# mayataka/idocp

Measured on AMD Instinct MI355X. Metric: SQP iterations/sec (whole node), higher is better.
Workload: dtype f64; 1 GPU; ANYmal OCPSolver N=100 T=5.05 FP64, trotting contact sequence (1 lift + 9 impulse events, 120 stages incl. impulse / aux / lift stages, switching constraints; BASELINE.json configs[2]); batch=1024 independent OCP instances per GPU, replicas across GPUs; horizon=100, batch_per_gpu=1024, parallelism=replicas x1

## Files before the change

### idocp_amd/csrc/ocp_nominal_kernel.hip

```cpp
#include <hip/hip_runtime.h>

#include "dev_dense.hpp"
#include "dev_lie.hpp"
#include "dev_rnea_tangent.hpp"
#include "ocp_device.hpp"
#include "ocp_launch.hpp"

namespace idocp_dev {

namespace {
using namespace rt;
__device__ __forceinline__ void st3g(double* __restrict__ p, V3 a) { p[0] = a.x; p[1] = a.y; p[2] = a.z; }
}

template <typename D, bool XYY, bool IMP>
__global__ __launch_bounds__(64) void ocp_nominal_kernel(OcpBuffers B, int dbg, int nlist, const double* __restrict__ q0) {
  using L = OcpLayout<D>;
  constexpr int NL = D::NL, LJ = D::LJ, NV = D::NV;
  constexpr int NOUT = 30, NIN = L::NJ_DYN - NOUT, TS = 31;
  __shared__ double tr[64 * TS];
  __shared__ long long recs[64];
  const OcpProblem* __restrict__ P = B.prob;
  const DevModel* __restrict__ m = B.model;
  const int M = B.M;
  const int lane = threadIdx.x;
  const int NTASK = 2 * NL + 1 + ((!IMP && q0 != nullptr) ? 3 : 0);
  const unsigned n_blk = blockIdx.x;
  const unsigned g_lo = n_blk & 7u, tg = n_blk >> 3;
  const unsigned g_hi = tg / NTASK;
  const int task = (int)(tg - g_hi * NTASK);
  const long unit = (long)(g_hi * 8u + g_lo) * 64 + lane;
  const int per = IMP ? nlist : M;
  const bool in_range = unit < (long)P->batch * per;
  const long b = in_range ? unit / per : 0;
  const int pos = in_range ? (IMP ? B.impulse_pos[(int)(unit - b * per)] : (int)(unit - b * per)) : (IMP ? B.impulse_pos[0] : 0);
  const OcpNode* __restrict__ nd = B.nodes + pos;
  const bool valid = in_range && pos != M - 1 && (IMP || nd->kind != 1);
  const long rec = (dbg & 2) ? 0 : b * B.NS + nd->slot;
  const double* __restrict__ s = B.sol + rec * L::SOL;
  double* __restrict__ nom = B.nom + rec * L::NOM;
  const double gz = IMP ? 0.0 : m->gravity[2];
  const double wv = 2.0 / P->baumgarte_time_step, wp = 1.0 / (P->baumgarte_time_step * P->baumgarte_time_step);
  const double* __restrict__ sq = s + L::S_Q;
  const double* __restrict__ sv = s + L::S_V;
  const double* __restrict__ sa = s + L::S_A;
  const double qx = sq[3], qy = sq[4], qz = sq[5], qw = sq[6];

  if (!IMP && task > 2 * NL) {
    if (!in_range) return;
    const int lt = task - 2 * NL - 1;
    double* __restrict__ zz = B.lie + rec * L::LIE;
    double R[9], p[3], Ja[36], Jb[36], d6[6];
    if (lt == 0) {
      lieRelative(B.q_ref + (long)pos * D::NQ, sq, R, p);
      lieLog6(R, p, d6);
      lieJlog6(R, p, Ja);
      for (int k = 0; k < 36; ++k) zz[L::Z_JQ + k] = Ja[k];
      for (int k = 0; k < 6; ++k) zz[L::Z_QDIFF + k] = d6[k];
    } else if (lt == 1) {
      if (pos == M - 1) return;
      lieRelative(B.sol + (b * B.NS + nd->next) * L::SOL + L::S_Q, sq, R, p);
      lieLog6(R, p, d6);
      lieJlog6(R, p, Ja);
      for (int k = 0; k < 36; ++k) zz[L::Z_FQQ + k] = Ja[k];
      for (int k = 0; k < 6; ++k) zz[L::Z_FQ6 + k] = d6[k];
      lieDDiffArg0(R, p, Ja, Jb);
      lieBlockInverse(Jb, Ja);
      for (int k = 0; k < 36; ++k) zz[L::Z_FQQI + k] = Ja[k];
    } else {
      const double* __restrict__ q_prev = (nd->prev < 0) ? (q0 + b * D::NQ) : (B.sol + (b * B.NS + nd->prev) * L::SOL + L::S_Q);
      lieRelative(sq, q_prev, R, p);
      lieJlog6(R, p, Ja);
      lieDDiffArg0(R, p, Ja, Jb);
      for (int k = 0; k < 36; ++k) zz[L::Z_FQQP + k] = Jb[k];
      lieBlockInverse(Jb, Ja);
      for (int k = 0; k < 36; ++k) zz[L::Z_FQQPI + k] = Ja[k];
    }
    return;
  }
  if (task <= NL) {
    const V3 zb = v3(2 * (qx * qz - qy * qw), 2 * (qy * qz + qx * qw), 1 - 2 * (qx * qx + qy * qy));
    V3 v = IMP ? ld3(sv) + ld3(sa) : ld3(sv), w = IMP ? ld3(sv + 3) + ld3(sa + 3) : ld3(sv + 3);
    V3 bl = ld3(sa) - gz * zb, bw = ld3(sa + 3);
    if (task == NL) {
      if (!valid) return;
      V3 hl = v3(0, 0, 0), hn = hl, f, n;
      const V3 mc = ld3(m->mc[0]);
      if (!IMP) inertia(m->mass[0], mc, m->Io[0], v, w, hl, hn);
      inertia(m->mass[0], mc, m->Io[0], bl, bw, f, n);
      double* br = nom + L::O_BASE;
      st3g(br + 0, zb); st3g(br + 3, v); st3g(br + 6, w); st3g(br + 9, hl); st3g(br + 12, hn); br[15] = 0.0;
      double* bn = nom + L::O_BN;
      if (IMP) { st3g(bn, f); st3g(bn + 3, n); }
      else { st3g(bn, f + cross(w, hl)); st3g(bn + 3, n + cross(w, hn) + cross(v, hl)); }
      double* idc = nom + L::O_IDC;
#pragma unroll
      for (int r = 0; r < 6; ++r) idc[r] = 0.0;
      for (int r = NV + nd->dimf; r < L::NVF; ++r) idc[r] = 0.0;
      return;
    }
    const int leg = task;
    recs[lane] = valid ? (long long)rec : -1;
    auto flush = [&](auto ncols, int offset) {
      constexpr int N = decltype(ncols)::value;
      waveLdsSync();
#pragma unroll 6
      for (int i = 0; i < N; ++i) {
        const int f = 64 * i + lane, st = f / N, k = f - st * N;
        const long long r = recs[st];
        if (r >= 0 && !(dbg & 1)) B.nom[r * L::NOM + offset + k] = tr[st * TS + k];
      }
      waveLdsSync();
    };
    double* my = tr + lane * TS;
    double Rj[LJ][12];
    V3 wj[LJ], vj[LJ], bwj[LJ], blj[LJ];
    V3 zc = zb;
#pragma unroll
    for (int j = 0; j < LJ; ++j) {
      const int ji = 1 + leg * LJ + j, dof = 6 + leg * LJ + j;
      double sj, cj;
      sincos(sq[dof + 1], &sj, &cj);
      Mat3<double> Rm;
      revoluteRotation<double>(m->R[ji], m->axis[ji], cj, sj, Rm);
#pragma unroll
      for (int e = 0; e < 9; ++e) Rj[j][e] = Rm.m[e];
      const V3 u = ld3(m->axis[ji]), p = ld3(m->p[ji]);
      st3(&Rj[j][9], u);
      const double qdd = sa[dof], qd = IMP ? sv[dof] + qdd : sv[dof];
      V3 wc, vc, bwc, blc, vJ;
      auto step = [&](auto tag) {
        const JointFrame<decltype(tag)::value> F(Rj[j], 0, 9);
        wc = F.mulT(w); vc = F.mulT(v + cross(w, p)); bwc = F.mulT(bw); blc = F.mulT(bl + cross(bw, p));
        zc = F.mulT(zc);
        vJ = F.timesU(qd);
        w = wc + vJ; v = vc;
        if constexpr (IMP) { bw = bwc + F.timesU(qdd); bl = blc; }
        else {
          bw = bwc + F.timesU(qdd) + F.crossKU(w, qd);
          bl = blc + F.crossKU(v, qd);
        }
      };
      if constexpr (XYY) { if (j == 0) step(AxisTag<0>{}); else step(AxisTag<1>{}); } else step(AxisTag<-1>{});
      wj[j] = w; vj[j] = v; bwj[j] = bw; blj[j] = bl;
#pragma unroll
      for (int e = 0; e < 9; ++e) my[e] = Rj[j][e];
      st3(my + 9, wc); st3(my + 12, vc); st3(my + 15, bwc); st3(my + 18, blc); st3(my + 21, zc); st3(my + 24, vJ); st3(my + 27, w);
      flush(AxisTag<NOUT>{}, L::O_JOINT + (leg * LJ + j) * L::NJ_DYN);
    }
    double* fr = nom + L::O_FEET + leg * L::NF_DYN;
    V3 fel = v3(0, 0, 0), fen = fel, fv = fel, fw = fel;
    double* idc = nom + L::O_IDC;
    if (valid && nd->active[leg]) {
      const double* __restrict__ Rc = P->contact_R[leg];
      const V3 pc = ld3(P->contact_p[leg]);
      const int row = NV + nd->row_of[leg];
      fv = XYY ? v + cross(w, pc) : mulT(Rc, v + cross(w, pc)); fw = XYY ? w : mulT(Rc, w);
      if constexpr (IMP) {
        idc[row] = fv.x; idc[row + 1] = fv.y; idc[row + 2] = fv.z;
      } else {
        const V3 fam = XYY ? bl + cross(bw, pc) : mulT(Rc, bl + cross(bw, pc));
        const V3 wxv = cross(fw, fv);
        idc[row] = fam.x + wxv.x + wv * fv.x;
        idc[row + 1] = fam.y + wxv.y + wv * fv.y;
        idc[row + 2] = fam.z + wxv.z + wv * fv.z;
      }
      fel = XYY ? ld3(s + L::S_F + 3 * leg) : mul(Rc, ld3(s + L::S_F + 3 * leg));
      fen = cross(pc, fel);
    }
    if (valid) { st3g(fr + 9, fv); st3g(fr + 12, fw); }
    V3 Fl = v3(0, 0, 0) - fel, Fn = v3(0, 0, 0) - fen;
#pragma unroll
    for (int j = LJ - 1; j >= 0; --j) {
      const int ji = 1 + leg * LJ + j, dof = 6 + leg * LJ + j;
      const V3 p = ld3(m->p[ji]), mc = ld3(m->mc[ji]);
      V3 hl = v3(0, 0, 0), hn = hl, f, n;
      inertia(m->mass[ji], mc, m->Io[ji], blj[j], bwj[j], f, n);
      if constexpr (IMP) { Fl = Fl + f; Fn = Fn + n; }
      else {
        inertia(m->mass[ji], mc, m->Io[ji], vj[j], wj[j], hl, hn);
        Fl = Fl + f + cross(wj[j], hl);
        Fn = Fn + n + cross(wj[j], hn) + cross(vj[j], hl);
      }
      st3(my, hl); st3(my + 3, hn); st3(my + 6, Fl); st3(my + 9, Fn);
      flush(AxisTag<NIN>{}, L::O_JOINT + (leg * LJ + j) * L::NJ_DYN + NOUT);
      auto back = [&](auto tag) {
        const JointFrame<decltype(tag)::value> F(Rj[j], 0, 9);
        if (valid) idc[dof] = F.dotU(Fn);
        const V3 Rf = F.mul(Fl);
        Fn = F.mul(Fn) + cross(p, Rf);
        Fl = Rf;
      };
      if constexpr (XYY) { if (j == 0) back(AxisTag<0>{}); else back(AxisTag<1>{}); } else back(AxisTag<-1>{});
    }
    if (valid) { double* bn = nom + L::O_BN + 6 * (1 + leg); st3g(bn, Fl); st3g(bn + 3, Fn); }
    return;
  }
  if (!valid) return;
  const int leg = task - NL - 1;
  double* fr = nom + L::O_FEET + leg * L::NF_DYN;
  V3 cp = v3(0, 0, 0);
  double rwc[9];
#pragma unroll
  for (int e = 0; e < 9; ++e) rwc[e] = 0.0;
  if (!IMP && nd->active[leg]) {
    double Rw[9];
    Rw[0] = 1 - 2 * (qy * qy + qz * qz); Rw[1] = 2 * (qx * qy - qz * qw);     Rw[2] = 2 * (qx * qz + qy * qw);
    Rw[3] = 2 * (qx * qy + qz * qw);     Rw[4] = 1 - 2 * (qx * qx + qz * qz); Rw[5] = 2 * (qy * qz - qx * qw);
    Rw[6] = 2 * (qx * qz - qy * qw);     Rw[7] = 2 * (qy * qz + qx * qw);     Rw[8] = 1 - 2 * (qx * qx + qy * qy);
    V3 pw = ld3(sq);
#pragma unroll
    for (int j = 0; j < LJ; ++j) {
      const int ji = 1 + leg * LJ + j, dof = 6 + leg * LJ + j;
      double sj, cj;
      sincos(sq[dof + 1], &sj, &cj);
      Mat3<double> Rm;
      revoluteRotation<double>(m->R[ji], m->axis[ji], cj, sj, Rm);
      pw = pw + mul(Rw, ld3(m->p[ji]));
      double Rl[12];
#pragma unroll
      for (int e = 0; e < 9; ++e) Rl[e] = Rm.m[e];
      st3(&Rl[9], ld3(m->axis[ji]));
      auto turn = [&](auto tag) {
        const JointFrame<decltype(tag)::value> F(Rl, 0, 9);
#pragma unroll
        for (int r = 0; r < 3; ++r) {
          const V3 row = F.mulT(v3(Rw[3 * r], Rw[3 * r + 1], Rw[3 * r + 2]));
          Rw[3 * r] = row.x; Rw[3 * r + 1] = row.y; Rw[3 * r + 2] = row.z;
        }
      };
      if constexpr (XYY) { if (j == 0) turn(AxisTag<0>{}); else turn(AxisTag<1>{}); } else turn(AxisTag<-1>{});
    }
    const double* __restrict__ Rc = P->contact_R[leg];
    const V3 pf = pw + mul(Rw, ld3(P->contact_p[leg]));
#pragma unroll
    for (int r = 0; r < 3; ++r)
#pragma unroll
      for (int c = 0; c < 3; ++c) rwc[3 * r + c] = XYY ? Rw[3 * r + c] : Rw[3 * r] * Rc[c] + Rw[3 * r + 1] * Rc[3 + c] + Rw[3 * r + 2] * Rc[6 + c];
    const V3 g = XYY ? gz * v3(Rw[6], Rw[7], Rw[8]) : mulT(Rc, gz * v3(Rw[6], Rw[7], Rw[8]));
    cp = v3(g.x + wp * (pf.x - nd->contact_point[leg][0]), g.y + wp * (pf.y - nd->contact_point[leg][1]),
            g.z + wp * (pf.z - nd->contact_point[leg][2]));
  }
#pragma unroll
  for (int e = 0; e < 9; ++e) fr[e] = rwc[e];
  st3g(fr + 15, cp);
}

template <typename D>
void OcpLaunch<D>::nominal(const OcpBuffers& B, long batch, int M, hipStream_t st, const double* q0_lie, hipStream_t st_imp) {
  const unsigned ntask = 2 * D::NL + 1 + (q0_lie ? 3 : 0);
  const unsigned groups = (unsigned)((batch * M + 63) / 64), blocks = ((groups + 7) / 8) * 8 * ntask;
  if (B.leg_axes_xyy) hipLaunchKernelGGL((ocp_nominal_kernel<D, true, false>), dim3(blocks), dim3(64), 0, st, B, 0, 0, q0_lie);
  else hipLaunchKernelGGL((ocp_nominal_kernel<D, false, false>), dim3(blocks), dim3(64), 0, st, B, 0, 0, q0_lie);
  if (B.n_impulse_fe > 0) {
    const unsigned gi = (unsigned)((batch * B.n_impulse_fe + 63) / 64), bi = ((gi + 7) / 8) * 8 * (2 * D::NL + 1);
    const double* none = nullptr;
    hipStream_t si = st_imp ? st_imp : st;
    if (B.leg_axes_xyy) hipLaunchKernelGGL((ocp_nominal_kernel<D, true, true>), dim3(bi), dim3(64), 0, si, B, 0, B.n_impulse_fe, none);
    else hipLaunchKernelGGL((ocp_nominal_kernel<D, false, true>), dim3(bi), dim3(64), 0, si, B, 0, B.n_impulse_fe, none);
  }
}

template void OcpLaunch<LeggedDims<4, 3>>::nominal(const OcpBuffers&, long, int, hipStream_t, const double*, hipStream_t);

}
```

Before: 212,500 SQP iterations/s.

## Coalesce nominal kernel loads/stores via LDS transposition and merge leg tasks

Loads of the per-stage solution (q, v, a, joint states, forces) and all scattered per-thread global stores (base record, feet, idc rows, Lie Jacobians) now go through a wave-level LDS transpose, so each wave issues contiguous loads and 16-byte stores. The separate foot-kinematics task is merged into the leg RNEA task, which cuts the task count from 2*NL+1 to NL+1 and removes duplicated sincos and rotation work. The price is more LDS traffic and barriers, higher register pressure in the merged leg task, and alignment static_asserts on the record layout.

```diff
diff --git a/idocp_amd/csrc/ocp_nominal_kernel.hip b/idocp_amd/csrc/ocp_nominal_kernel.hip
--- a/idocp_amd/csrc/ocp_nominal_kernel.hip
+++ b/idocp_amd/csrc/ocp_nominal_kernel.hip
@@ -10,21 +10,56 @@
 
 namespace {
 using namespace rt;
-__device__ __forceinline__ void st3g(double* __restrict__ p, V3 a) { p[0] = a.x; p[1] = a.y; p[2] = a.z; }
+
+template <int S, int N, bool W16>
+__device__ __forceinline__ void trStore(const double* col0, const int* recs, unsigned long long live, double* __restrict__ out, int reclen, int offset, int lane) {
+  static_assert(!W16 || N % 2 == 0, "16-byte runs have an even length");
+  constexpr int W = W16 ? 2 : 1, NW = N / W;
+#pragma unroll 6
+  for (int i = 0; i < NW; ++i) {
+    const int e = 64 * i + lane, st = e / NW, k = W * (e - st * NW);
+    if (!((live >> st) & 1ull)) continue;
+    double* __restrict__ dst = out + (long)recs[st] * reclen + offset + k;
+    if constexpr (W16) *reinterpret_cast<double2*>(dst) = make_double2(col0[st * S + k], col0[st * S + k + 1]);
+    else *dst = col0[st * S + k];
+  }
+}
+template <int S, int N>
+__device__ __forceinline__ void trStoreAt(const double* col0, const int* recs, const int* at, unsigned long long live, double* __restrict__ out, int reclen, int offset, int lane) {
+#pragma unroll
+  for (int i = 0; i < N; ++i) {
+    const int e = 64 * i + lane, st = e / N, k = e - st * N;
+    if (((live >> st) & 1ull) && at[st] >= 0) out[(long)recs[st] * reclen + offset + at[st] + k] = col0[st * S + k];
+  }
+}
+template <int S, int N>
+__device__ __forceinline__ void trLoad(double* col0, const int* recs, const double* __restrict__ in, int reclen, int offset, int lane) {
+#pragma unroll
+  for (int i = 0; i < N; ++i) {
+    const int e = 64 * i + lane, st = e / N, k = e - st * N;
+    col0[st * S + k] = in[(long)recs[st] * reclen + offset + k];
+  }
+}
 }
 
 template <typename D, bool XYY, bool IMP>
 __global__ __launch_bounds__(64) void ocp_nominal_kernel(OcpBuffers B, int dbg, int nlist, const double* __restrict__ q0) {
   using L = OcpLayout<D>;
-  constexpr int NL = D::NL, LJ = D::LJ, NV = D::NV;
+  constexpr int NL = D::NL, LJ = D::LJ, NV = D::NV, NF = D::NF;
   constexpr int NOUT = 30, NIN = L::NJ_DYN - NOUT, TS = 31;
-  __shared__ double tr[64 * TS];
-  __shared__ long long recs[64];
+  static_assert(L::NOM % 2 == 0 && L::LIE % 2 == 0 && L::O_JOINT % 2 == 0 && L::NJ_DYN % 2 == 0 && NOUT % 2 == 0 && L::O_FEET % 2 == 0 && L::NF_DYN % 2 == 0 &&
+                L::O_BASE % 2 == 0 && L::NB_DYN % 2 == 0 && L::O_BN % 2 == 0, "16-byte stores of the nominal record");
+  static_assert(L::Z_JQ % 2 == 0 && L::Z_FQQ % 2 == 0 && L::Z_FQQI % 2 == 0 && L::Z_FQQP % 2 == 0, "16-byte stores of the Lie record");
+  static_assert(L::Z_QDIFF == L::Z_JQ + 36 && L::Z_FQ6 == L::Z_FQQ + 36 && L::Z_FQQPI == L::Z_FQQP + 36, "neighbouring Lie blocks leave as one run");
+  static_assert(L::O_BN == L::O_BASE + L::NB_DYN && L::NB_DYN == 16, "base record and own base force leave as one run");
+  static_assert(L::NF_DYN == 18 && 16 + 3 * LJ <= TS && L::NF_DYN + 3 <= TS && 6 + LJ <= TS, "rows of the leg task");
+  __shared__ __attribute__((aligned(16))) double tr[64 * TS];
+  __shared__ int recs[64], aux[64];
   const OcpProblem* __restrict__ P = B.prob;
   const DevModel* __restrict__ m = B.model;
   const int M = B.M;
   const int lane = threadIdx.x;
-  const int NTASK = 2 * NL + 1 + ((!IMP && q0 != nullptr) ? 3 : 0);
+  const int NTASK = NL + 1 + ((!IMP && q0 != nullptr) ? 3 : 0);
   const unsigned n_blk = blockIdx.x;
   const unsigned g_lo = n_blk & 7u, tg = n_blk >> 3;
   const unsigned g_hi = tg / NTASK;
@@ -37,223 +72,266 @@
   const OcpNode* __restrict__ nd = B.nodes + pos;
   const bool valid = in_range && pos != M - 1 && (IMP || nd->kind != 1);
   const long rec = (dbg & 2) ? 0 : b * B.NS + nd->slot;
-  const double* __restrict__ s = B.sol + rec * L::SOL;
-  double* __restrict__ nom = B.nom + rec * L::NOM;
+  const unsigned long long store_on = (dbg & 1) ? 0ull : ~0ull;
   const double gz = IMP ? 0.0 : m->gravity[2];
   const double wv = 2.0 / P->baumgarte_time_step, wp = 1.0 / (P->baumgarte_time_step * P->baumgarte_time_step);
-  const double* __restrict__ sq = s + L::S_Q;
-  const double* __restrict__ sv = s + L::S_V;
-  const double* __restrict__ sa = s + L::S_A;
-  const double qx = sq[3], qy = sq[4], qz = sq[5], qw = sq[6];
-
-  if (!IMP && task > 2 * NL) {
-    if (!in_range) return;
-    const int lt = task - 2 * NL - 1;
-    double* __restrict__ zz = B.lie + rec * L::LIE;
+  recs[lane] = (int)rec;
+  double* my = tr + lane * TS;
+  auto put = [&](auto k0_, auto n_, auto get, unsigned long long live, double* __restrict__ out, int reclen, int offset) {
+    constexpr int K0 = decltype(k0_)::value, N = decltype(n_)::value, S = N | 1;
+    static_assert(N <= TS - 1 && K0 % 2 == 0, "a block fits the transposition; runs stay 16-byte aligned");
+#pragma unroll
+    for (int k = 0; k < N; ++k) tr[lane * S + k] = get(K0 + k);
+    waveLdsSync();
+    trStore<S, N, true>(tr, recs, live, out, reclen, offset + K0, lane);
+    waveLdsSync();
+  };
+
+  if (!IMP && task > NL) {
+    const int lt = task - NL - 1;
+    constexpr int SQ = 7;
+    waveLdsSync();
+    trLoad<SQ, 7>(tr, recs, B.sol, L::SOL, L::S_Q, lane);
+    waveLdsSync();
+    double sq[7];
+#pragma unroll
+    for (int k = 0; k < 7; ++k) sq[k] = tr[lane * SQ + k];
+    waveLdsSync();
     double R[9], p[3], Ja[36], Jb[36], d6[6];
+    auto JaD6 = [&](int k) { return k < 36 ? Ja[k] : d6[k - 36]; };
+    auto JaOnly = [&](int k) { return Ja[k]; };
+    auto JbJa = [&](int k) { return k < 36 ? Jb[k] : Ja[k - 36]; };
     if (lt == 0) {
+      const unsigned long long live = __ballot(in_range) & store_on;
       lieRelative(B.q_ref + (long)pos * D::NQ, sq, R, p);
       lieLog6(R, p, d6);
       lieJlog6(R, p, Ja);
-      for (int k = 0; k < 36; ++k) zz[L::Z_JQ + k] = Ja[k];
-      for (int k = 0; k < 6; ++k) zz[L::Z_QDIFF + k] = d6[k];
+      put(AxisTag<0>{}, AxisTag<22>{}, JaD6, live, B.lie, L::LIE, L::Z_JQ);
+      put(AxisTag<22>{}, AxisTag<20>{}, JaD6, live, B.lie, L::LIE, L::Z_JQ);
     } else if (lt == 1) {
-      if (pos == M - 1) return;
-      lieRelative(B.sol + (b * B.NS + nd->next) * L::SOL + L::S_Q, sq, R, p);
+      const bool on = in_range && pos != M - 1;
+      const unsigned long long live = __ballot(on) & store_on;
+      lieRelative(B.sol + (b * B.NS + (on ? nd->next : nd->slot)) * L::SOL + L::S_Q, sq, R, p);
       lieLog6(R, p, d6);
       lieJlog6(R, p, Ja);
-      for (int k = 0; k < 36; ++k) zz[L::Z_FQQ + k] = Ja[k];
-      for (int k = 0; k < 6; ++k) zz[L::Z_FQ6 + k] = d6[k];
+      put(AxisTag<0>{}, AxisTag<22>{}, JaD6, live, B.lie, L::LIE, L::Z_FQQ);
+      put(AxisTag<22>{}, AxisTag<20>{}, JaD6, live, B.lie, L::LIE, L::Z_FQQ);
       lieDDiffArg0(R, p, Ja, Jb);
       lieBlockInverse(Jb, Ja);
-      for (int k = 0; k < 36; ++k) zz[L::Z_FQQI + k] = Ja[k];
+      put(AxisTag<0>{}, AxisTag<18>{}, JaOnly, live, B.lie, L::LIE, L::Z_FQQI);
+      put(AxisTag<18>{}, AxisTag<18>{}, JaOnly, live, B.lie, L::LIE, L::Z_FQQI);
     } else {
+      const unsigned long long live = __ballot(in_range) & store_on;
       const double* __restrict__ q_prev = (nd->prev < 0) ? (q0 + b * D::NQ) : (B.sol + (b * B.NS + nd->prev) * L::SOL + L::S_Q);
       lieRelative(sq, q_prev, R, p);
       lieJlog6(R, p, Ja);
       lieDDiffArg0(R, p, Ja, Jb);
-      for (int k = 0; k < 36; ++k) zz[L::Z_FQQP + k] = Jb[k];
       lieBlockInverse(Jb, Ja);
-      for (int k = 0; k < 36; ++k) zz[L::Z_FQQPI + k] = Ja[k];
+      put(AxisTag<0>{}, AxisTag<24>{}, JbJa, live, B.lie, L::LIE, L::Z_FQQP);
+      put(AxisTag<24>{}, AxisTag<24>{}, JbJa, live, B.lie, L::LIE, L::Z_FQQP);
+      put(AxisTag<48>{}, AxisTag<24>{}, JbJa, live, B.lie, L::LIE, L::Z_FQQP);
     }
     return;
   }
-  if (task <= NL) {
-    const V3 zb = v3(2 * (qx * qz - qy * qw), 2 * (qy * qz + qx * qw), 1 - 2 * (qx * qx + qy * qy));
-    V3 v = IMP ? ld3(sv) + ld3(sa) : ld3(sv), w = IMP ? ld3(sv + 3) + ld3(sa + 3) : ld3(sv + 3);
-    V3 bl = ld3(sa) - gz * zb, bw = ld3(sa + 3);
-    if (task == NL) {
-      if (!valid) return;
-      V3 hl = v3(0, 0, 0), hn = hl, f, n;
-      const V3 mc = ld3(m->mc[0]);
-      if (!IMP) inertia(m->mass[0], mc, m->Io[0], v, w, hl, hn);
-      inertia(m->mass[0], mc, m->Io[0], bl, bw, f, n);
-      double* br = nom + L::O_BASE;
-      st3g(br + 0, zb); st3g(br + 3, v); st3g(br + 6, w); st3g(br + 9, hl); st3g(br + 12, hn); br[15] = 0.0;
-      double* bn = nom + L::O_BN;
-      if (IMP) { st3g(bn, f); st3g(bn + 3, n); }
-      else { st3g(bn, f + cross(w, hl)); st3g(bn + 3, n + cross(w, hn) + cross(v, hl)); }
-      double* idc = nom + L::O_IDC;
-#pragma unroll
-      for (int r = 0; r < 6; ++r) idc[r] = 0.0;
-      for (int r = NV + nd->dimf; r < L::NVF; ++r) idc[r] = 0.0;
-      return;
-    }
-    const int leg = task;
-    recs[lane] = valid ? (long long)rec : -1;
-    auto flush = [&](auto ncols, int offset) {
-      constexpr int N = decltype(ncols)::value;
-      waveLdsSync();
-#pragma unroll 6
-      for (int i = 0; i < N; ++i) {
-        const int f = 64 * i + lane, st = f / N, k = f - st * N;
-        const long long r = recs[st];
-        if (r >= 0 && !(dbg & 1)) B.nom[r * L::NOM + offset + k] = tr[st * TS + k];
-      }
-      waveLdsSync();
-    };
-    double* my = tr + lane * TS;
-    double Rj[LJ][12];
-    V3 wj[LJ], vj[LJ], bwj[LJ], blj[LJ];
-    V3 zc = zb;
-#pragma unroll
-    for (int j = 0; j < LJ; ++j) {
-      const int ji = 1 + leg * LJ + j, dof = 6 + leg * LJ + j;
-      double sj, cj;
-      sincos(sq[dof + 1], &sj, &cj);
-      Mat3<double> Rm;
-      revoluteRotation<double>(m->R[ji], m->axis[ji], cj, sj, Rm);
-#pragma unroll
-      for (int e = 0; e < 9; ++e) Rj[j][e] = Rm.m[e];
-      const V3 u = ld3(m->axis[ji]), p = ld3(m->p[ji]);
-      st3(&Rj[j][9], u);
-      const double qdd = sa[dof], qd = IMP ? sv[dof] + qdd : sv[dof];
-      V3 wc, vc, bwc, blc, vJ;
-      auto step = [&](auto tag) {
-        const JointFrame<decltype(tag)::value> F(Rj[j], 0, 9);
-        wc = F.mulT(w); vc = F.mulT(v + cross(w, p)); bwc = F.mulT(bw); blc = F.mulT(bl + cross(bw, p));
-        zc = F.mulT(zc);
-        vJ = F.timesU(qd);
-        w = wc + vJ; v = vc;
-        if constexpr (IMP) { bw = bwc + F.timesU(qdd); bl = blc; }
-        else {
-          bw = bwc + F.timesU(qdd) + F.crossKU(w, qd);
-          bl = blc + F.crossKU(v, qd);
-        }
-      };
-      if constexpr (XYY) { if (j == 0) step(AxisTag<0>{}); else step(AxisTag<1>{}); } else step(AxisTag<-1>{});
-      wj[j] = w; vj[j] = v; bwj[j] = bw; blj[j] = bl;
-#pragma unroll
-      for (int e = 0; e < 9; ++e) my[e] = Rj[j][e];
-      st3(my + 9, wc); st3(my + 12, vc); st3(my + 15, bwc); st3(my + 18, blc); st3(my + 21, zc); st3(my + 24, vJ); st3(my + 27, w);
-      flush(AxisTag<NOUT>{}, L::O_JOINT + (leg * LJ + j) * L::NJ_DYN);
-    }
-    double* fr = nom + L::O_FEET + leg * L::NF_DYN;
-    V3 fel = v3(0, 0, 0), fen = fel, fv = fel, fw = fel;
-    double* idc = nom + L::O_IDC;
-    if (valid && nd->active[leg]) {
-      const double* __restrict__ Rc = P->contact_R[leg];
-      const V3 pc = ld3(P->contact_p[leg]);
-      const int row = NV + nd->row_of[leg];
-      fv = XYY ? v + cross(w, pc) : mulT(Rc, v + cross(w, pc)); fw = XYY ? w : mulT(Rc, w);
-      if constexpr (IMP) {
-        idc[row] = fv.x; idc[row + 1] = fv.y; idc[row + 2] = fv.z;
-      } else {
-        const V3 fam = XYY ? bl + cross(bw, pc) : mulT(Rc, bl + cross(bw, pc));
-        const V3 wxv = cross(fw, fv);
-        idc[row] = fam.x + wxv.x + wv * fv.x;
-        idc[row + 1] = fam.y + wxv.y + wv * fv.y;
-        idc[row + 2] = fam.z + wxv.z + wv * fv.z;
-      }
-      fel = XYY ? ld3(s + L::S_F + 3 * leg) : mul(Rc, ld3(s + L::S_F + 3 * leg));
-      fen = cross(pc, fel);
-    }
-    if (valid) { st3g(fr + 9, fv); st3g(fr + 12, fw); }
-    V3 Fl = v3(0, 0, 0) - fel, Fn = v3(0, 0, 0) - fen;
-#pragma unroll
-    for (int j = LJ - 1; j >= 0; --j) {
-      const int ji = 1 + leg * LJ + j, dof = 6 + leg * LJ + j;
-      const V3 p = ld3(m->p[ji]), mc = ld3(m->mc[ji]);
-      V3 hl = v3(0, 0, 0), hn = hl, f, n;
-      inertia(m->mass[ji], mc, m->Io[ji], blj[j], bwj[j], f, n);
-      if constexpr (IMP) { Fl = Fl + f; Fn = Fn + n; }
-      else {
-        inertia(m->mass[ji], mc, m->Io[ji], vj[j], wj[j], hl, hn);
-        Fl = Fl + f + cross(wj[j], hl);
-        Fn = Fn + n + cross(wj[j], hn) + cross(vj[j], hl);
-      }
-      st3(my, hl); st3(my + 3, hn); st3(my + 6, Fl); st3(my + 9, Fn);
-      flush(AxisTag<NIN>{}, L::O_JOINT + (leg * LJ + j) * L::NJ_DYN + NOUT);
-      auto back = [&](auto tag) {
-        const JointFrame<decltype(tag)::value> F(Rj[j], 0, 9);
-        if (valid) idc[dof] = F.dotU(Fn);
-        const V3 Rf = F.mul(Fl);
-        Fn = F.mul(Fn) + cross(p, Rf);
-        Fl = Rf;
-      };
-      if constexpr (XYY) { if (j == 0) back(AxisTag<0>{}); else back(AxisTag<1>{}); } else back(AxisTag<-1>{});
-    }
-    if (valid) { double* bn = nom + L::O_BN + 6 * (1 + leg); st3g(bn, Fl); st3g(bn + 3, Fn); }
+  const unsigned long long live = __ballot(valid) & store_on;
+  const int leg = task < NL ? task : 0;
+  constexpr int C_V = 7, C_A = 13, C_QJ = 19, C_VJ = C_QJ + LJ, C_AJ = C_VJ + LJ, C_F = C_AJ + LJ;
+  waveLdsSync();
+  trLoad<TS, 7>(tr, recs, B.sol, L::SOL, L::S_Q, lane);
+  trLoad<TS, 6>(tr + C_V, recs, B.sol, L::SOL, L::S_V, lane);
+  trLoad<TS, 6>(tr + C_A, recs, B.sol, L::SOL, L::S_A, lane);
+  if (task < NL) {
+    trLoad<TS, LJ>(tr + C_QJ, recs, B.sol, L::SOL, L::S_Q + 7 + leg * LJ, lane);
+    trLoad<TS, LJ>(tr + C_VJ, recs, B.sol, L::SOL, L::S_V + 6 + leg * LJ, lane);
+    trLoad<TS, LJ>(tr + C_AJ, recs, B.sol, L::SOL, L::S_A + 6 + leg * LJ, lane);
+    trLoad<TS, 3>(tr + C_F, recs, B.sol, L::SOL, L::S_F + 3 * leg, lane);
+  }
+  waveLdsSync();
+  double sq[7], sv[6], sa[6];
+#pragma unroll
+  for (int k = 0; k < 7; ++k) sq[k] = my[k];
+#pragma unroll
+  for (int k = 0; k < 6; ++k) { sv[k] = my[C_V + k]; sa[k] = my[C_A + k]; }
+  const double qx = sq[3], qy = sq[4], qz = sq[5], qw = sq[6];
+  const V3 zb = v3(2 * (qx * qz - qy * qw), 2 * (qy * qz + qx * qw), 1 - 2 * (qx * qx + qy * qy));
+  V3 v = IMP ? ld3(sv) + ld3(sa) : ld3(sv), w = IMP ? ld3(sv + 3) + ld3(sa + 3) : ld3(sv + 3);
+  V3 bl = ld3(sa) - gz * zb, bw = ld3(sa + 3);
+  if (task == NL) {
+    waveLdsSync();
+    V3 hl = v3(0, 0, 0), hn = hl, f, n;
+    const V3 mc = ld3(m->mc[0]);
+    if (!IMP) inertia(m->mass[0], mc, m->Io[0], v, w, hl, hn);
+    inertia(m->mass[0], mc, m->Io[0], bl, bw, f, n);
+    constexpr int SB = (L::NB_DYN + 6) | 1;
+    double* br = tr + lane * SB;
+    st3(br + 0, zb); st3(br + 3, v); st3(br + 6, w); st3(br + 9, hl); st3(br + 12, hn); br[15] = 0.0;
+    double* bn = br + L::NB_DYN;
+    if (IMP) { st3(bn, f); st3(bn + 3, n); }
+    else { st3(bn, f + cross(w, hl)); st3(bn + 3, n + cross(w, hn) + cross(v, hl)); }
+    aux[lane] = nd->dimf;
+    waveLdsSync();
+    trStore<SB, L::NB_DYN + 6, true>(tr, recs, live, B.nom, L::NOM, L::O_BASE, lane);
+#pragma unroll
+    for (int i = 0; i < 6; ++i) {
+      const int e = 64 * i + lane, st = e / 6, k = e - st * 6;
+      if ((live >> st) & 1ull) B.nom[(long)recs[st] * L::NOM + L::O_IDC + k] = 0.0;
+    }
+#pragma unroll
+    for (int i = 0; i < NF; ++i) {
+      const int e = 64 * i + lane, st = e / NF, k = e - st * NF;
+      if (((live >> st) & 1ull) && k >= aux[st]) B.nom[(long)recs[st] * L::NOM + L::O_IDC + NV + k] = 0.0;
+    }
     return;
   }
-  if (!valid) return;
-  const int leg = task - NL - 1;
-  double* fr = nom + L::O_FEET + leg * L::NF_DYN;
-  V3 cp = v3(0, 0, 0);
-  double rwc[9];
-#pragma unroll
-  for (int e = 0; e < 9; ++e) rwc[e] = 0.0;
-  if (!IMP && nd->active[leg]) {
-    double Rw[9];
+  double qj[LJ], qdj[LJ], qddj[LJ];
+#pragma unroll
+  for (int j = 0; j < LJ; ++j) { qj[j] = my[C_QJ + j]; qdj[j] = my[C_VJ + j]; qddj[j] = my[C_AJ + j]; }
+  const V3 fs = ld3(my + C_F);
+  waveLdsSync();
+  auto flush = [&](auto ncols, int offset) {
+    constexpr int N = decltype(ncols)::value;
+    waveLdsSync();
+    trStore<TS, N, true>(tr, recs, live, B.nom, L::NOM, offset, lane);
+    waveLdsSync();
+  };
+  double Rj[LJ][12];
+  V3 wj[LJ], vj[LJ], bwj[LJ], blj[LJ];
+  V3 zc = zb;
+  double Rw[9];
+  V3 pw = ld3(sq);
+  if constexpr (!IMP) {
     Rw[0] = 1 - 2 * (qy * qy + qz * qz); Rw[1] = 2 * (qx * qy - qz * qw);     Rw[2] = 2 * (qx * qz + qy * qw);
     Rw[3] = 2 * (qx * qy + qz * qw);     Rw[4] = 1 - 2 * (qx * qx + qz * qz); Rw[5] = 2 * (qy * qz - qx * qw);
     Rw[6] = 2 * (qx * qz - qy * qw);     Rw[7] = 2 * (qy * qz + qx * qw);     Rw[8] = 1 - 2 * (qx * qx + qy * qy);
-    V3 pw = ld3(sq);
-#pragma unroll
-    for (int j = 0; j < LJ; ++j) {
-      const int ji = 1 + leg * LJ + j, dof = 6 + leg * LJ + j;
-      double sj, cj;
-      sincos(sq[dof + 1], &sj, &cj);
-      Mat3<double> Rm;
-      revoluteRotation<double>(m->R[ji], m->axis[ji], cj, sj, Rm);
-      pw = pw + mul(Rw, ld3(m->p[ji]));
-      double Rl[12];
-#pragma unroll
-      for (int e = 0; e < 9; ++e) Rl[e] = Rm.m[e];
-      st3(&Rl[9], ld3(m->axis[ji]));
-      auto turn = [&](auto tag) {
-        const JointFrame<decltype(tag)::value> F(Rl, 0, 9);
+  }
+#pragma unroll
+  for (int j = 0; j < LJ; ++j) {
+    const int ji = 1 + leg * LJ + j;
+    double sj, cj;
+    sincos(qj[j], &sj, &cj);
+    Mat3<double> Rm;
+    revoluteRotation<double>(m->R[ji], m->axis[ji], cj, sj, Rm);
+#pragma unroll
+    for (int e = 0; e < 9; ++e) Rj[j][e] = Rm.m[e];
+    const V3 u = ld3(m->axis[ji]), p = ld3(m->p[ji]);
+    st3(&Rj[j][9], u);
+    const double qdd = qddj[j], qd = IMP ? qdj[j] + qdd : qdj[j];
+    V3 wc, vc, bwc, blc, vJ;
+    if constexpr (!IMP) pw = pw + mul(Rw, p);
+    auto step = [&](auto tag) {
+      const JointFrame<decltype(tag)::value> F(Rj[j], 0, 9);
+      wc = F.mulT(w); vc = F.mulT(v + cross(w, p)); bwc = F.mulT(bw); blc = F.mulT(bl + cross(bw, p));
+      zc = F.mulT(zc);
+      vJ = F.timesU(qd);
+      w = wc + vJ; v = vc;
+      if constexpr (IMP) { bw = bwc + F.timesU(qdd); bl = blc; }
+      else {
+        bw = bwc + F.timesU(qdd) + F.crossKU(w, qd);
+        bl = blc + F.crossKU(v, qd);
 #pragma unroll
         for (int r = 0; r < 3; ++r) {
           const V3 row = F.mulT(v3(Rw[3 * r], Rw[3 * r + 1], Rw[3 * r + 2]));
           Rw[3 * r] = row.x; Rw[3 * r + 1] = row.y; Rw[3 * r + 2] = row.z;
         }
-      };
-      if constexpr (XYY) { if (j == 0) turn(AxisTag<0>{}); else turn(AxisTag<1>{}); } else turn(AxisTag<-1>{});
-    }
+      }
+    };
+    if constexpr (XYY) { if (j == 0) step(AxisTag<0>{}); else step(AxisTag<1>{}); } else step(AxisTag<-1>{});
+    wj[j] = w; vj[j] = v; bwj[j] = bw; blj[j] = bl;
+#pragma unroll
+    for (int e = 0; e < 9; ++e) my[e] = Rj[j][e];
+    st3(my + 9, wc); st3(my + 12, vc); st3(my + 15, bwc); st3(my + 18, blc); st3(my + 21, zc); st3(my + 24, vJ); st3(my + 27, w);
+    flush(AxisTag<NOUT>{}, L::O_JOINT + (leg * LJ + j) * L::NJ_DYN);
+  }
+  V3 fel = v3(0, 0, 0), fen = fel, fv = fel, fw = fel, crow = fel;
+  const bool act = nd->active[leg];
+  if (valid && act) {
     const double* __restrict__ Rc = P->contact_R[leg];
-    const V3 pf = pw + mul(Rw, ld3(P->contact_p[leg]));
-#pragma unroll
-    for (int r = 0; r < 3; ++r)
-#pragma unroll
-      for (int c = 0; c < 3; ++c) rwc[3 * r + c] = XYY ? Rw[3 * r + c] : Rw[3 * r] * Rc[c] + Rw[3 * r + 1] * Rc[3 + c] + Rw[3 * r + 2] * Rc[6 + c];
-    const V3 g = XYY ? gz * v3(Rw[6], Rw[7], Rw[8]) : mulT(Rc, gz * v3(Rw[6], Rw[7], Rw[8]));
-    cp = v3(g.x + wp * (pf.x - nd->contact_point[leg][0]), g.y + wp * (pf.y - nd->contact_point[leg][1]),
-            g.z + wp * (pf.z - nd->contact_point[leg][2]));
-  }
-#pragma unroll
-  for (int e = 0; e < 9; ++e) fr[e] = rwc[e];
-  st3g(fr + 15, cp);
+    const V3 pc = ld3(P->contact_p[leg]);
+    fv = XYY ? v + cross(w, pc) : mulT(Rc, v + cross(w, pc)); fw = XYY ? w : mulT(Rc, w);
+    if constexpr (IMP) {
+      crow = fv;
+    } else {
+      const V3 fam = XYY ? bl + cross(bw, pc) : mulT(Rc, bl + cross(bw, pc));
+      const V3 wxv = cross(fw, fv);
+      crow = v3(fam.x + wxv.x + wv * fv.x, fam.y + wxv.y + wv * fv.y, fam.z + wxv.z + wv * fv.z);
+    }
+    fel = XYY ? fs : mul(Rc, fs);
+    fen = cross(pc, fel);
+  }
+  V3 cp = v3(0, 0, 0);
+  double rwc[9];
+#pragma unroll
+  for (int e = 0; e < 9; ++e) rwc[e] = 0.0;
+  if constexpr (!IMP) {
+    if (act) {
+      const double* __restrict__ Rc = P->contact_R[leg];
+      const V3 pf = pw + mul(Rw, ld3(P->contact_p[leg]));
+#pragma unroll
+      for (int r = 0; r < 3; ++r)
+#pragma unroll
+        for (int c = 0; c < 3; ++c) rwc[3 * r + c] = XYY ? Rw[3 * r + c] : Rw[3 * r] * Rc[c] + Rw[3 * r + 1] * Rc[3 + c] + Rw[3 * r + 2] * Rc[6 + c];
+      const V3 g = XYY ? gz * v3(Rw[6], Rw[7], Rw[8]) : mulT(Rc, gz * v3(Rw[6], Rw[7], Rw[8]));
+      cp = v3(g.x + wp * (pf.x - nd->contact_point[leg][0]), g.y + wp * (pf.y - nd->contact_point[leg][1]),
+              g.z + wp * (pf.z - nd->contact_point[leg][2]));
+    }
+  }
+  {
+    constexpr int SF = (L::NF_DYN + 3) | 1;
+    double* fr = tr + lane * SF;
+#pragma unroll
+    for (int e = 0; e < 9; ++e) fr[e] = rwc[e];
+    st3(fr + 9, fv); st3(fr + 12, fw); st3(fr + 15, cp); st3(fr + L::NF_DYN, crow);
+    aux[lane] = (valid && act) ? NV + nd->row_of[leg] : -1;
+    waveLdsSync();
+    trStore<SF, L::NF_DYN, true>(tr, recs, live, B.nom, L::NOM, L::O_FEET + leg * L::NF_DYN, lane);
+    trStoreAt<SF, 3>(tr + L::NF_DYN, recs, aux, live, B.nom, L::NOM, L::O_IDC, lane);
+    waveLdsSync();
+  }
+  V3 Fl = v3(0, 0, 0) - fel, Fn = v3(0, 0, 0) - fen;
+  double tau[LJ];
+#pragma unroll
+  for (int j = LJ - 1; j >= 0; --j) {
+    const int ji = 1 + leg * LJ + j;
+    const V3 p = ld3(m->p[ji]), mc = ld3(m->mc[ji]);
+    V3 hl = v3(0, 0, 0), hn = hl, f, n;
+    inertia(m->mass[ji], mc, m->Io[ji], blj[j], bwj[j], f, n);
+    if constexpr (IMP) { Fl = Fl + f; Fn = Fn + n; }
+    else {
+      inertia(m->mass[ji], mc, m->Io[ji], vj[j], wj[j], hl, hn);
+      Fl = Fl + f + cross(wj[j], hl);
+      Fn = Fn + n + cross(wj[j], hn) + cross(vj[j], hl);
+    }
+    st3(my, hl); st3(my + 3, hn); st3(my + 6, Fl); st3(my + 9, Fn);
+    flush(AxisTag<NIN>{}, L::O_JOINT + (leg * LJ + j) * L::NJ_DYN + NOUT);
+    auto back = [&](auto tag) {
+      const JointFrame<decltype(tag)::value> F(Rj[j], 0, 9);
+      tau[j] = F.dotU(Fn);
+      const V3 Rf = F.mul(Fl);
+      Fn = F.mul(Fn) + cross(p, Rf);
+      Fl = Rf;
+    };
+    if constexpr (XYY) { if (j == 0) back(AxisTag<0>{}); else back(AxisTag<1>{}); } else back(AxisTag<-1>{});
+  }
+  {
+    constexpr int SN = (6 + LJ) | 1;
+    double* bn = tr + lane * SN;
+    st3(bn, Fl); st3(bn + 3, Fn);
+#pragma unroll
+    for (int j = 0; j < LJ; ++j) bn[6 + j] = tau[j];
+    waveLdsSync();
+    trStore<SN, 6, true>(tr, recs, live, B.nom, L::NOM, L::O_BN + 6 * (1 + leg), lane);
+    trStore<SN, LJ, false>(tr + 6, recs, live, B.nom, L::NOM, L::O_IDC + 6 + leg * LJ, lane);
+  }
 }
 
 template <typename D>
 void OcpLaunch<D>::nominal(const OcpBuffers& B, long batch, int M, hipStream_t st, const double* q0_lie, hipStream_t st_imp) {
-  const unsigned ntask = 2 * D::NL + 1 + (q0_lie ? 3 : 0);
+  const unsigned ntask = D::NL + 1 + (q0_lie ? 3 : 0);
   const unsigned groups = (unsigned)((batch * M + 63) / 64), blocks = ((groups + 7) / 8) * 8 * ntask;
   if (B.leg_axes_xyy) hipLaunchKernelGGL((ocp_nominal_kernel<D, true, false>), dim3(blocks), dim3(64), 0, st, B, 0, 0, q0_lie);
   else hipLaunchKernelGGL((ocp_nominal_kernel<D, false, false>), dim3(blocks), dim3(64), 0, st, B, 0, 0, q0_lie);
   if (B.n_impulse_fe > 0) {
-    const unsigned gi = (unsigned)((batch * B.n_impulse_fe + 63) / 64), bi = ((gi + 7) / 8) * 8 * (2 * D::NL + 1);
+    const unsigned gi = (unsigned)((batch * B.n_impulse_fe + 63) / 64), bi = ((gi + 7) / 8) * 8 * (D::NL + 1);
     const double* none = nullptr;
     hipStream_t si = st_imp ? st_imp : st;
     if (B.leg_axes_xyy) hipLaunchKernelGGL((ocp_nominal_kernel<D, true, true>), dim3(bi), dim3(64), 0, si, B, 0, B.n_impulse_fe, none);
```

Result: no change. 214,100 SQP iterations/s (median of 6 runs) (+0.7%).
